# PhiFEM/phiFEM

Measured on AMD Instinct MI355X. Metric: assembled+solved DoF/s, 3D Poisson phi-FEM (tag+assemble+solve), higher is better.
Workload: dtype f64

## Files before the change

include/phifem_hip.h:

```cpp
#ifndef PHIFEM_HIP_H
#define PHIFEM_HIP_H

#include <stdint.h>

#ifdef __cplusplus
extern "C" {
#endif

typedef struct phx_mesh phx_mesh;
typedef struct phx_system phx_system;

enum phx_status {
  PHX_OK = 0,
  PHX_ERR_VALUE = -1,
  PHX_ERR_NOT_IMPLEMENTED = -2,
  PHX_ERR_HIP = -3,
  PHX_ERR_PARTITION = -4,
  PHX_ERR_CAPACITY = -5,
  PHX_ERR_BREAKDOWN = -6,
  PHX_ERR_TIMEOUT = -7
};

enum phx_loc { PHX_HOST = 0, PHX_DEVICE = 1 };

// ... 15 lines not shown
  PHX_ARR_BFACETS = 6,
  PHX_ARR_C2E = 7,
  PHX_ARR_EDGES = 8
};

int phx_version(void);
const char *phx_last_error(void);
int phx_device_count(int *n);
int phx_pool_release(void);
int phx_pool_stats(int64_t *live_bytes, int64_t *cached_bytes);

int phx_detection_points(int cell_type, int degree, int which, double *out, int64_t *npts);

int phx_levelset_points_count(phx_mesh *m, int detection_degree, int64_t *count);
int phx_levelset_eval_points(phx_mesh *m, int detection_degree, const double *nodal, int loc,
                             double *out_device);
int phx_detection_points_physical(phx_mesh *m, int detection_degree, double *out_device);

int phx_lagrange_nodes(int cell_type, int degree, double *out, int64_t *n);
int phx_lagrange_tabulate(int cell_type, int degree, int64_t npts, const double *pts, double *out);
int phx_levelset_eval_points_deg(phx_mesh *m, int detection_degree, int levelset_degree, const double *nodal,
                                 int loc, double *out_device);
int phx_lagrange_dof_points(phx_mesh *m, int degree, double *out_device);

int phx_topology_build_host(int cell_type, int64_t nv, int64_t nc, const int32_t *cells,
                            int32_t *c2f, int32_t *f2c, int64_t *nf);

int phx_mesh_create(int gdim, int cell_type, int64_t nv, const double *coords, int64_t nc,
                    const int32_t *cells, int device, phx_mesh **out);

int phx_mesh_create_box(int gdim, const double *lo, const double *hi, const int64_t *n,
                        const int64_t *offset, const int64_t *n_global, int device,
                        phx_mesh **out);

int phx_mesh_set_slab_faces(phx_mesh *m, int lower_is_cut, int upper_is_cut);
int phx_mesh_destroy(phx_mesh *m);
int phx_mesh_edge_count(phx_mesh *m, int64_t *ne);
int phx_mesh_counts(const phx_mesh *m, int64_t *counts);
int phx_mesh_get_array(phx_mesh *m, int which, void *out, int loc);
int phx_mesh_stream(phx_mesh *m, uint64_t *stream);
int phx_mesh_synchronize(phx_mesh *m);
int phx_mesh_set_stream(phx_mesh *m, uint64_t stream);
enum phx_option {
  PHX_OPT_PROFILE_SPMV = 1,
  PHX_OPT_HAS_EXTERIOR = 2,
  PHX_OPT_SPMV_XCD_GROUP = 3,
  PHX_OPT_PRECOND = 5,
  PHX_OPT_EXPORT_CSR = 7,
  PHX_OPT_STRUCTURED = 8,
  PHX_OPT_DETERMINISTIC = 9,
  PHX_OPT_EL_COARSE = 10,
  PHX_OPT_STENCIL_PLANE_ROWS = 11,
  PHX_OPT_P2_COARSE = 12,
  PHX_OPT_ALLOW_EMPTY = 6,
  PHX_OPT_SPMV_VALUE_INDEX = 4
};
int phx_set_option(phx_mesh *m, int option, int64_t value);
int phx_box_poisson_solve(int device, const int *L, const double *h, int f32, double *f_host);
int phx_box_dst_bench(int device, const int *L, int f32, int reps, double *out_us3);
int phx_dense_inverse(int device, int64_t n, double *a_host, int *singular);
int phx_event_pair_overhead(phx_mesh *m, double *seconds);
int phx_mesh_tag_histogram(const phx_mesh *m, int64_t *cells4, int64_t *facets7);

int phx_tag_cells(phx_mesh *m, int phi_kind, const double *phi, int loc, int detection_degree,
                  int single_layer_cut, int *warn_zero_denominator);

int phx_tag_facets(phx_mesh *m, int phi_kind, const double *phi, int loc, int detection_degree);

int phx_overwrite_tags(phx_mesh *m, int entity_is_facet, int64_t n, const int32_t *indices,
                       const int32_t *values);
int phx_set_tags(phx_mesh *m, int entity_is_facet, const int32_t *values, int loc);

int phx_integration_entities(phx_mesh *m, int which, int32_t *out, int64_t *n_pairs);

int phx_submesh_create(phx_mesh *m, phx_mesh **sub);
int phx_submesh_maps(phx_mesh *sub, int32_t *c_map, int32_t *v_map);

int phx_partition_cells(phx_mesh *m, int nparts, const int32_t *weights, int32_t *part, int loc);
int phx_partition_layout(phx_mesh *m, int nparts, const int32_t *part, int rank, int32_t *owner, uint8_t *flags, int loc);
int phx_submesh_create_from_flags(phx_mesh *m, const uint8_t *flags, int loc, phx_mesh **sub);

int phx_mesh_refine(phx_mesh *m, phx_mesh **fine);
int phx_prolongate(phx_mesh *coarse, phx_mesh *fine, int degree, int ncomp, const double *in, int loc_in,
                   double *out, int loc_out);
int phx_refine_tables(int cell_type, int32_t *children, int *nchild, double *p2_weights);

int phx_locate_points(phx_mesh *m, int64_t npts, const double *pts, int loc, double tol, int32_t *cells_out,
                      double *xref_out, int loc_out);
int phx_eval_points(phx_mesh *m, int degree, int ncomp, const double *values, int loc_v, int64_t npts,
                    const int32_t *cells, const double *xref, int loc_p, int want_grad, double fill, double *out,
                    double *grad_out, int loc_out);
int phx_locator_info(const phx_mesh *m, int64_t *info);
int phx_locate_timings(const phx_mesh *m, double *t);

int phx_assemble_poisson_wd(phx_mesh *m, double pen_coef, double stab_coef, const double *phi_h,
                            const double *f_h, const double *u_D, int loc, phx_system **out);
int phx_assemble_poisson_wd_p2(phx_mesh *m, double pen_coef, double stab_coef, const double *phi_h,
                               int phi_degree, const double *f_h, const double *u_D, int loc,
                               phx_system **out);
int phx_assemble_poisson_sd(phx_mesh *m, double stab_coef, int degree, const double *phi_h,
                            int phi_degree, const double *f_h, int loc, phx_system **out);
int phx_assemble_poisson_flux(phx_mesh *m, const double *params, int facet_tag, int quadrature_degree,
                              const double *phi_h, const double *f_h, const double *g_h, int loc,
                              phx_system **out);
int phx_assemble_elasticity_if(phx_mesh *m, const double *params, const double *phi_h,
                               const double *f_h, const double *u_D, const int32_t *bc_vertices,
// ... 61 lines not shown
```

phifem_amd/_lib.py:

```python
import ctypes as C
import os

_HERE = os.path.dirname(os.path.abspath(__file__))
LIB_PATH = os.path.join(_HERE, "libphifem_hip.so")

if not os.path.exists(LIB_PATH):
    raise ImportError(
        f"{LIB_PATH} is missing: build it with `python -c 'import __graft_entry__ as g; g.build()'` "
        "(or `make -C phifem_amd/csrc`).  phifem_amd has no CPU fallback.")

if os.environ.get("PHIFEM_NO_TORCH", "") != "1":
    try:
        import torch
    except ImportError:
        pass

lib = C.CDLL(LIB_PATH)

HOST, DEVICE = 0, 1
TRIANGLE, QUADRILATERAL, TETRAHEDRON = 0, 1, 2
CELL_TYPES = {"triangle": TRIANGLE, "quadrilateral": QUADRILATERAL, "tetrahedron": TETRAHEDRON}
CELL_NAMES = {v: k for k, v in CELL_TYPES.items()}
PHI_NODAL_P1, PHI_POINTS, PHI_QUADRIC = 0, 1, 2
(OPT_PROFILE_SPMV, OPT_HAS_EXTERIOR, OPT_SPMV_XCD_GROUP, OPT_SPMV_VALUE_INDEX, OPT_PRECOND, OPT_ALLOW_EMPTY,
 OPT_EXPORT_CSR, OPT_STRUCTURED, OPT_DETERMINISTIC, OPT_EL_COARSE, OPT_STENCIL_PLANE_ROWS, OPT_P2_COARSE) = (
    1, 2, 3, 4, 5, 6, 7, 8, 9, 10, 11, 12)
(ARR_COORDS, ARR_CELLS, ARR_C2F, ARR_F2C, ARR_CELL_TAGS, ARR_FACET_TAGS, ARR_BFACETS, ARR_C2E,
 ARR_EDGES) = range(9)

OK, ERR_VALUE, ERR_NOT_IMPLEMENTED, ERR_HIP, ERR_PARTITION, ERR_CAPACITY, ERR_BREAKDOWN, ERR_TIMEOUT = (
    0, -1, -2, -3, -4, -5, -6, -7)

_vp, _i, _i64, _d = C.c_void_p, C.c_int, C.c_int64, C.c_double
_pi, _pi64, _pd = C.POINTER(C.c_int), C.POINTER(C.c_int64), C.POINTER(C.c_double)

SIGNATURES = {
    "phx_version": ([], _i),
    "phx_last_error": ([], C.c_char_p),
    "phx_device_count": ([_pi], _i),
    "phx_pool_release": ([], _i),
    "phx_pool_stats": ([_pi64, _pi64], _i),
    "phx_detection_points": ([_i, _i, _i, _vp, _pi64], _i),
    "phx_levelset_points_count": ([_vp, _i, _pi64], _i),
    "phx_levelset_eval_points": ([_vp, _i, _vp, _i, _vp], _i),
    "phx_detection_points_physical": ([_vp, _i, _vp], _i),
    "phx_lagrange_nodes": ([_i, _i, _vp, _pi64], _i),
    "phx_lagrange_tabulate": ([_i, _i, _i64, _vp, _vp], _i),
    "phx_levelset_eval_points_deg": ([_vp, _i, _i, _vp, _i, _vp], _i),
    "phx_lagrange_dof_points": ([_vp, _i, _vp], _i),
    "phx_topology_build_host": ([_i, _i64, _i64, _vp, _vp, _vp, _pi64], _i),
    "phx_mesh_create": ([_i, _i, _i64, _vp, _i64, _vp, _i, C.POINTER(_vp)], _i),
    "phx_mesh_create_box": ([_i, _vp, _vp, _vp, _vp, _vp, _i, C.POINTER(_vp)], _i),
    "phx_mesh_set_slab_faces": ([_vp, _i, _i], _i),
    "phx_mesh_destroy": ([_vp], _i),
    "phx_mesh_counts": ([_vp, _pi64], _i),
    "phx_mesh_edge_count": ([_vp, _pi64], _i),
    "phx_mesh_get_array": ([_vp, _i, _vp, _i], _i),
    "phx_mesh_stream": ([_vp, C.POINTER(C.c_uint64)], _i),
    "phx_mesh_synchronize": ([_vp], _i),
    "phx_mesh_set_stream": ([_vp, C.c_uint64], _i),
    "phx_set_option": ([_vp, _i, _i64], _i),
    "phx_event_pair_overhead": ([_vp, _pd], _i),
    "phx_box_poisson_solve": ([_i, _pi, _pd, _i, _vp], _i),
    "phx_box_dst_bench": ([_i, _pi, _i, _i, _pd], _i),
    "phx_mesh_tag_histogram": ([_vp, _pi64, _pi64], _i),
    "phx_krylov_precond_active": ([_vp, _pi], _i),
    "phx_krylov_precond_disable": ([_vp], _i),
    "phx_precond_info": ([_vp, _pd], _i),
    "phx_coarse_info": ([_vp, _pd], _i),
    "phx_coarse_export": ([_vp, _vp, _vp], _i),
    "phx_precond_local_bbox": ([_vp, _pi64], _i),
    "phx_precond_setup_global": ([_vp, _pi64, _i, _i, _pi64, _pi64], _i),
    "phx_precond_set_carry_buffers": ([_vp, _vp, _vp], _i),
    "phx_precond_dist_info": ([_vp, _pi64], _i),
    "phx_krylov_attach": ([_vp, _vp, _vp, _vp], _i),
    "phx_krylov_phase": ([_vp, _i], _i),
    "phx_krylov_finish": ([_vp, _vp, _i], _i),
    "phx_krylov_profile": ([_vp, _i, _pd, _pi64], _i),
    "phx_system_get_perm": ([_vp, _vp, _vp, _vp, _i], _i),
# ... 96 lines not shown
```

phifem_amd/csrc/phx_common.h:

```cpp
#pragma once
#include <hip/hip_runtime.h>
#include <stdint.h>
#include <stdio.h>
#include <string>
#include <vector>

#include "../../include/phifem_hip.h"
#include "phx_switches.h"

#define PHX_MAX_PTS 40
#define PHX_MAX_VPC 4

void phx_set_error(const char *fmt, ...);

hipError_t phx_pool_malloc(void **p, size_t bytes);
hipError_t phx_pool_free(void *p);
void phx_pool_trim(void);
template <typename T>
static inline hipError_t phx_malloc(T **p, size_t bytes) { return phx_pool_malloc((void **)p, bytes); }
static inline hipError_t phx_free(void *p) { return phx_pool_free(p); }

#define PHX_HIP(expr)                                                                       \
  do {                                                                                      \
    hipError_t e_ = (expr);                                                                 \
// ... 57 lines not shown
  int32_t *bfacets = nullptr;
  int32_t *bfacet_ids = nullptr;
  uint8_t *facet_exempt = nullptr;
  bool slab_cut = false;
  int64_t ne = 0;
  int32_t *c2e = nullptr;
  int32_t *edges = nullptr;
  bool c2e_is_alias = false;
  int64_t box_n[3] = {0, 0, 0};
  double box_h[3] = {0.0, 0.0, 0.0};
  int64_t box_off[3] = {0, 0, 0};
  int64_t box_nglob[3] = {0, 0, 0};
  double box_lo[3] = {0.0, 0.0, 0.0}, box_hi[3] = {0.0, 0.0, 0.0};
  int64_t *v2c_ptr = nullptr;
  int32_t *v2c_idx = nullptr;
  bool is_box = false;
  int64_t box_plane = 0, box_nlast = 0;
  int8_t *cell_tags = nullptr;
  int8_t *facet_tags = nullptr;
  bool have_cell_tags = false, have_facet_tags = false;
  int64_t tag_hist[4] = {0, 0, 0, 0};
  int64_t ftag_hist[8] = {0, 0, 0, 0, 0, 0, 0, 0};
  int32_t *sel_counts[2] = {nullptr, nullptr};
  bool sel_counts_valid = false;
  int64_t sel_total[2] = {0, 0};
  int32_t *sel_counts_cut = nullptr;
  bool sel_cut_valid = false;
  uint8_t *act_in = nullptr, *act_cut = nullptr;
  bool act_valid = false;
  int64_t *ent_buf[2] = {nullptr, nullptr};
  int64_t ent_count[2] = {0, 0};
  bool have_entities = false;
  bool is_submesh = false;
  int32_t *c_map_h = nullptr, *v_map_h = nullptr;
  bool on_box_lattice = false;
  int32_t *v2lat = nullptr;
  int32_t *lat2v = nullptr;
  double timings[8] = {0, 0, 0, 0, 0, 0, 0, 0};
  struct phx_locator *locator = nullptr;
  int rect_checked = 0;
  double loc_timings[3] = {0, 0, 0};
  bool own_stream = true;
  int profile_spmv = 0;
  int spmv_xcd_group = 0;
  int64_t stencil_plane_rows = 32768;
  int spmv_value_index = 1;
  int precond = 1;
  int has_exterior_override = -1;
  std::vector<hipEvent_t> prof_ev[2];
  int prof_used[2] = {0, 0}, prof_seen[2] = {0, 0};
  double *scal_h = nullptr;
  int export_csr = 0;
  int structured = 1;
  int allow_empty = 0;
  int el_coarse = -1;
  int p2_coarse = 0;
  int deterministic = 0;
  phx_mesh *inner = nullptr;
  int32_t *in_cmap = nullptr;
  int32_t *in_fmap = nullptr;
};

struct phx_p2_lattice {
  int64_t n[3];
  int64_t F[3];
  int64_t nv;
  int64_t base[8];
  int64_t ext[7][3];
};
__host__ __device__ __forceinline__ int phx_p2_edge_class(int a, int b, int c) {
  const int nd = a + b + c;
  return nd == 1 ? (a ? 0 : (b ? 1 : 2)) : (nd == 2 ? (!c ? 3 : (!b ? 4 : 5)) : 6);
}
__host__ __device__ __forceinline__ int64_t phx_p2_entity_of_fine(const phx_p2_lattice &L, int64_t I, int64_t J, int64_t K) {
  const int a = (int)(I & 1), b = (int)(J & 1), c = (int)(K & 1);
  const int64_t i = I >> 1, j = J >> 1, k = K >> 1;
  if (!(a | b | c)) return i + (L.n[0] + 1) * (j + (L.n[1] + 1) * k);
  const int cls = phx_p2_edge_class(a, b, c);
  return L.nv + L.base[cls] + i + L.ext[cls][0] * (j + L.ext[cls][1] * k);
}
__host__ __device__ __forceinline__ void phx_p2_fine_of_entity(const phx_p2_lattice &L, int64_t e, int64_t *q) {
  if (e < L.nv) {
    const int64_t n0 = L.n[0] + 1, n1 = L.n[1] + 1, r = e / n0;
    q[0] = 2 * (e - r * n0); q[1] = 2 * (r % n1); q[2] = 2 * (r / n1);
    return;
  }
  const int64_t id = e - L.nv;
  int cls = 0;
  while (cls < 6 && id >= L.base[cls + 1]) ++cls;
  const int64_t rem = id - L.base[cls], r = rem / L.ext[cls][0];
  const int dir[7][3] = {{1, 0, 0}, {0, 1, 0}, {0, 0, 1}, {1, 1, 0}, {1, 0, 1}, {0, 1, 1}, {1, 1, 1}};
  q[0] = 2 * (rem - r * L.ext[cls][0]) + dir[cls][0];
  q[1] = 2 * (r % L.ext[cls][1]) + dir[cls][1];
  q[2] = 2 * (r / L.ext[cls][1]) + dir[cls][2];
}
#define PHX_P2S_REC 32
struct phx_p2_struct {
  phx_p2_lattice lat;
  double *coef = nullptr;
  unsigned long long *mask = nullptr;
  double *tabE = nullptr, *tabO = nullptr;
  unsigned *linemask = nullptr;
  int32_t *runs = nullptr;
  int64_t nrun = 0, nc0i = 0;
};

// ... 109 lines not shown
```

phifem_amd/csrc/phx_mesh.hip:

```cpp
#include "phx_prim.h"
#include <stdarg.h>
#include <string.h>

#include <algorithm>
#include <atomic>
#include <vector>

#include "phx_common.h"
#include "phx_select.h"

static thread_local char g_err[1024] = "";

void phx_set_error(const char *fmt, ...) {
  va_list ap;
  va_start(ap, fmt);
  vsnprintf(g_err, sizeof(g_err), fmt, ap);
  va_end(ap);
}

#include <map>
#include <mutex>
#include <unordered_map>
namespace {
struct Pool {
// ... 1059 lines not shown
  }
  RbArgs a;
  memset(&a, 0, sizeof(a));
  a.n = n;
  int tot = 0;
  for (int i = 0; i < n; ++i) {
    PHX_REQUIRE(items[i].bytes > 0 && items[i].bytes <= 64, PHX_ERR_VALUE, "read-back item of %d bytes", items[i].bytes);
    a.src[i] = static_cast<const uint8_t *>(items[i].dev);
    a.bytes[i] = items[i].bytes;
    a.off[i] = tot;
    tot += (items[i].bytes + 7) & ~7;
  }
  k_rb_pack<<<1, 64, 0, st>>>(a, sg.dev);
  PHX_HIP(hipGetLastError());
  PHX_HIP(hipMemcpyAsync(sg.pin, sg.dev, (size_t)tot, hipMemcpyDeviceToHost, st));
  PHX_HIP(hipStreamSynchronize(st));
  for (int i = 0; i < n; ++i) memcpy(items[i].host, sg.pin + a.off[i], (size_t)items[i].bytes);
  return PHX_OK;
}

int phx_mesh_pinned_scalars(phx_mesh *m, double **out) {
  if (!m->scal_h) PHX_HIP(hipHostMalloc(&m->scal_h, sizeof(double) * 16));
  *out = m->scal_h;
  return PHX_OK;
}

extern "C" int phx_mesh_stream(phx_mesh *m, uint64_t *stream) {
  *stream = (uint64_t)(uintptr_t)m->stream;
  return PHX_OK;
}

extern "C" int phx_mesh_set_stream(phx_mesh *m, uint64_t stream) {
  PHX_HIP(hipSetDevice(m->device));
  PHX_HIP(hipStreamSynchronize(m->stream));
  if (m->own_stream) PHX_HIP(hipStreamDestroy(m->stream));
  m->stream = (hipStream_t)(uintptr_t)stream;
  m->own_stream = false;
  if (m->inner) m->inner->stream = m->stream;
  return PHX_OK;
}

extern "C" int phx_set_option(phx_mesh *m, int option, int64_t value) {
  if (m->inner) PHX_CHECK(phx_set_option(m->inner, option, value));
  switch (option) {
    case PHX_OPT_PROFILE_SPMV:
      PHX_REQUIRE(value >= 0 && value <= 1024, PHX_ERR_VALUE, "SpMV profiling stride out of range");
      m->profile_spmv = (int)value;
      return PHX_OK;
    case PHX_OPT_HAS_EXTERIOR: m->has_exterior_override = (int)value; return PHX_OK;
    case PHX_OPT_SPMV_VALUE_INDEX: m->spmv_value_index = value != 0; return PHX_OK;
    case PHX_OPT_ALLOW_EMPTY: m->allow_empty = value != 0; return PHX_OK;
    case PHX_OPT_EXPORT_CSR: m->export_csr = value != 0; return PHX_OK;
    case PHX_OPT_STRUCTURED: m->structured = value != 0; return PHX_OK;
    case PHX_OPT_DETERMINISTIC: m->deterministic = value != 0; return PHX_OK;
    case PHX_OPT_EL_COARSE:
      PHX_REQUIRE(value == -1 || value == 0 || (value >= 5 && value <= 4096), PHX_ERR_VALUE, "coarse ratio %lld: -1, 0 or >= 5", (long long)value);
      m->el_coarse = (int)value;
      return PHX_OK;
    case PHX_OPT_P2_COARSE:
      PHX_REQUIRE(value == -1 || value == 0 || (value >= 5 && value <= 4096), PHX_ERR_VALUE, "coarse ratio %lld: -1, 0 or >= 5", (long long)value);
      m->p2_coarse = (int)value;
      return PHX_OK;
    case PHX_OPT_PRECOND:
      PHX_REQUIRE(value >= 0 && value <= 2, PHX_ERR_VALUE, "unknown preconditioner %lld", (long long)value);
      m->precond = (int)value;
      return PHX_OK;
    case PHX_OPT_SPMV_XCD_GROUP:
      PHX_REQUIRE(value >= 0 && value < (1 << 24), PHX_ERR_VALUE, "XCD group size out of range");
      m->spmv_xcd_group = (int)value;
      return PHX_OK;
    case PHX_OPT_STENCIL_PLANE_ROWS:
      PHX_REQUIRE(value >= 0, PHX_ERR_VALUE, "rows per plane out of range");
      m->stencil_plane_rows = value;
      return PHX_OK;
    default: phx_set_error("unknown option %d", option); return PHX_ERR_VALUE;
  }
}

extern "C" int phx_mesh_tag_histogram(const phx_mesh *m, int64_t *cells4, int64_t *facets7) {
  if (cells4) for (int i = 0; i < 4; ++i) cells4[i] = m->tag_hist[i];
  if (facets7) for (int i = 0; i < 7; ++i) facets7[i] = m->ftag_hist[i];
  return PHX_OK;
}

extern "C" int phx_mesh_synchronize(phx_mesh *m) {
  PHX_HIP(hipSetDevice(m->device));
  PHX_HIP(hipStreamSynchronize(m->stream));
  return PHX_OK;
}

__global__ void k_widen_tags(int64_t n, const int8_t *__restrict__ in, int32_t *__restrict__ out) {
  const int64_t i = blockIdx.x * (int64_t)blockDim.x + threadIdx.x;
  if (i < n) out[i] = (int32_t)(in[i] & PHX_TAG_MASK);
}

extern "C" int phx_mesh_get_array(phx_mesh *m, int which, void *out, int loc) {
  PHX_HIP(hipSetDevice(m->device));
  const hipMemcpyKind kind = loc == PHX_DEVICE ? hipMemcpyDeviceToDevice : hipMemcpyDeviceToHost;
  const void *src = nullptr;
  size_t bytes = 0;
  switch (which) {
    case PHX_ARR_COORDS: src = m->x; bytes = sizeof(double) * m->nv * m->gdim; break;
    case PHX_ARR_CELLS: src = m->cells; bytes = sizeof(int32_t) * m->nc * m->ci.nvpc; break;
    case PHX_ARR_C2F: src = m->c2f; bytes = sizeof(int32_t) * m->nc * m->ci.nfpc; break;
    case PHX_ARR_F2C: src = m->f2c; bytes = sizeof(int32_t) * m->nf * 2; break;
    case PHX_ARR_BFACETS: src = m->bfacets; bytes = sizeof(int32_t) * m->nbf * 2; break;
// ... 36 lines not shown
```

phifem_amd/csrc/phx_tag.hip:

```cpp
#include "phx_prim.h"
#include <string.h>

#include <algorithm>
#include <vector>

#include "phx_common.h"
#include "phx_select.h"

int phx_shape_table(int cell_type, int degree, int which, std::vector<double> &tab, int *npts,
                    int *nfun);

struct DetTab {
  int npts, nfun;
  double N[PHX_MAX_PTS * 4];
};
struct Quadric {
  double c[3], s[3], c0;
};
struct FacetVerts {
  int nfpc, nvpf;
  int fv[4][3];
};

template <int GDIM>
// ... 323 lines not shown
  unsigned long long a = 0;
  for (int64_t i = blockIdx.x * (int64_t)blockDim.x + threadIdx.x; i < nblocks; i += (int64_t)gridDim.x * blockDim.x)
    a += part[(size_t)b * nblocks + i];
  red[threadIdx.x] = a;
  __syncthreads();
  for (int o = 128; o > 0; o >>= 1) {
    if ((int)threadIdx.x < o) red[threadIdx.x] += red[threadIdx.x + o];
    __syncthreads();
  }
  if (threadIdx.x == 0 && red[0]) atomicAdd(&hist[b], red[0]);
}

struct SelTag34 {
  const int8_t *ft;
  __host__ __device__ bool operator()(const int32_t &f) const { return ft[f] == 3 || ft[f] == 4; }
  __host__ __device__ const int8_t *bytes() const { return ft; }
  __host__ __device__ bool test(int t, int32_t) const { return t == 3 || t == 4; }
};

template <bool FILL>
__global__ void k_entities(int64_t nlist, const int32_t *__restrict__ list,
                           const int32_t *__restrict__ f2c, const int32_t *__restrict__ c2f,
                           int nfpc, const int8_t *__restrict__ ctags,
                           const int8_t *__restrict__ ftags, int32_t *__restrict__ cnt0,
                           int32_t *__restrict__ cnt1, const int32_t *__restrict__ off0,
                           const int32_t *__restrict__ off1, int64_t *__restrict__ out0,
                           int64_t *__restrict__ out1) {
  const int64_t i = blockIdx.x * (int64_t)blockDim.x + threadIdx.x;
  if (i >= nlist) return;
  const int64_t f = list[i];
  const int w = ftags[f] == 4 ? 0 : 1;
  const int cell_mask = w == 0 ? ((1 << 1) | (1 << 2)) : ((1 << 2) | (1 << 3));
  const int32_t c0 = f2c[2 * f], c1 = f2c[2 * f + 1];
  int n = 0;
  for (int pos = 0; pos < 2; ++pos) {
    const int32_t c = c1 >= 0 ? (pos == 0 ? c1 : c0) : (pos == 0 ? c0 : -1);
    if (c < 0) continue;
    const int t = ctags[c] & PHX_TAG_MASK;
    if (t > 30 || !((cell_mask >> t) & 1)) continue;
    if (FILL) {
      int lf = 0;
      for (int k = 0; k < nfpc; ++k)
        if (c2f[(int64_t)c * nfpc + k] == (int32_t)f) lf = k;
      int64_t *out = w == 0 ? out0 : out1;
      const int64_t slot = (w == 0 ? off0[i] : off1[i]) + n;
      out[2 * slot] = 2 * f + pos;
      out[2 * slot + 1] = ((int64_t)c << 8) | lf;
    }
    ++n;
  }
  if (!FILL) { cnt0[i] = w == 0 ? n : 0; cnt1[i] = w == 1 ? n : 0; }
}

static int make_tab(const phx_mesh *m, int degree, int which, DetTab *tab) {
  std::vector<double> t;
  int npts = 0, nfun = 0;
  PHX_CHECK(phx_shape_table(m->cell_type, degree, which, t, &npts, &nfun));
  memset(tab, 0, sizeof(*tab));
  tab->npts = npts;
  tab->nfun = nfun;
  for (size_t i = 0; i < t.size(); ++i) tab->N[i] = t[i];
  return PHX_OK;
}

static int stage_phi(phx_mesh *m, int phi_kind, const double *phi, int loc, int64_t count,
                     const double **dev, double **owned, Quadric *quad) {
  *owned = nullptr;
  *dev = nullptr;
  memset(quad, 0, sizeof(*quad));
  PHX_REQUIRE(phi != nullptr, PHX_ERR_VALUE, "phi is NULL");
  if (phi_kind == PHX_PHI_QUADRIC) {
    double h[7];
    if (loc == PHX_DEVICE) PHX_HIP(hipMemcpy(h, phi, sizeof(h), hipMemcpyDeviceToHost));
    else memcpy(h, phi, sizeof(h));
    for (int a = 0; a < 3; ++a) { quad->c[a] = h[a]; quad->s[a] = h[3 + a]; }
    quad->c0 = h[6];
    return PHX_OK;
  }
  if (loc == PHX_DEVICE) { *dev = phi; return PHX_OK; }
  PHX_HIP(phx_malloc(owned, sizeof(double) * (size_t)(count > 0 ? count : 1)));
  PHX_HIP(hipMemcpyAsync(*owned, phi, sizeof(double) * (size_t)count, hipMemcpyHostToDevice, m->stream));
  *dev = *owned;
  return PHX_OK;
}

static int64_t cell_points_count(const phx_mesh *m, int degree) {
  DetTab t;
  if (make_tab(m, degree, 0, &t) != PHX_OK) return 0;
  return t.npts;
}

static int read_hist(phx_mesh *m, const int8_t *tags, int64_t n, int nbins, int64_t *out, const void *extra = nullptr,
                     size_t extra_bytes = 0, void *extra_host = nullptr) {
  unsigned long long *d = nullptr;
  PHX_HIP(phx_malloc(&d, sizeof(unsigned long long) * 8));
  PHX_HIP(hipMemsetAsync(d, 0, sizeof(unsigned long long) * 8, m->stream));
  const int blocks = (int)std::min<int64_t>(phx_div_up(n, 256), 2048);
  k_tag_hist<<<dim3(blocks), dim3(256), 0, m->stream>>>(n, tags, nbins, d);
  unsigned long long h[8];
  const phx_rb_item rb[2] = {{d, (int)sizeof(h), h}, {extra, (int)extra_bytes, extra_host}};
  PHX_CHECK(phx_read_back(m->stream, rb, extra ? 2 : 1));
  PHX_HIP(phx_free(d));
  for (int i = 0; i < nbins; ++i) out[i] = (int64_t)h[i];
  return PHX_OK;
}

template <int KIND>
static int launch_tag_cells(phx_mesh *m, const DetTab &tab, const double *dphi, const Quadric &q,
                            int *dwarn) {
  const dim3 grid((unsigned)phx_div_up(m->nc, 256)), block(256);
  if (m->cell_type == PHX_TRIANGLE)
    k_tag_cells<KIND, 2, 3><<<grid, block, 0, m->stream>>>(m->nc, tab, m->cells, dphi, m->x, q, m->cell_tags, dwarn);
  else if (m->cell_type == PHX_QUADRILATERAL)
    k_tag_cells<KIND, 2, 4><<<grid, block, 0, m->stream>>>(m->nc, tab, m->cells, dphi, m->x, q, m->cell_tags, dwarn);
  else
    k_tag_cells<KIND, 3, 4><<<grid, block, 0, m->stream>>>(m->nc, tab, m->cells, dphi, m->x, q, m->cell_tags, dwarn);
  PHX_HIP(hipGetLastError());
  return PHX_OK;
}

extern "C" int phx_tag_cells(phx_mesh *m, int phi_kind, const double *phi, int loc,
                             int detection_degree, int single_layer_cut,
                             int *warn_zero_denominator) {
  PHX_HIP(hipSetDevice(m->device));
  PHX_REQUIRE(phi_kind >= 0 && phi_kind <= 2, PHX_ERR_VALUE, "unknown phi_kind %d", phi_kind);
  DetTab tab;
  PHX_CHECK(make_tab(m, detection_degree, 0, &tab));
  const double *dphi = nullptr;
  double *owned = nullptr;
  Quadric quad;
  const int64_t count = phi_kind == PHX_PHI_NODAL_P1 ? m->nv : m->nc * (int64_t)tab.npts;
  PHX_CHECK(stage_phi(m, phi_kind, phi, loc, count, &dphi, &owned, &quad));
  int *dwarn = nullptr;
  PHX_HIP(phx_malloc(&dwarn, sizeof(int)));
  PHX_HIP(hipMemsetAsync(dwarn, 0, sizeof(int), m->stream));
  PHX_CHECK(phx_begin_timing(m));
  if (phi_kind == PHX_PHI_NODAL_P1) PHX_CHECK(launch_tag_cells<PHX_PHI_NODAL_P1>(m, tab, dphi, quad, dwarn));
  else if (phi_kind == PHX_PHI_POINTS) PHX_CHECK(launch_tag_cells<PHX_PHI_POINTS>(m, tab, dphi, quad, dwarn));
  else PHX_CHECK(launch_tag_cells<PHX_PHI_QUADRIC>(m, tab, dphi, quad, dwarn));
  uint8_t *touched = nullptr, *vcut = nullptr;
  const dim3 grid4((unsigned)phx_div_up(phx_div_up(m->nc, 4), 256)), block4(256);
  m->act_valid = false;
  if (single_layer_cut) {
    if (!m->act_in) PHX_HIP(phx_malloc(&m->act_in, (size_t)m->nv));
    if (!m->act_cut) PHX_HIP(phx_malloc(&m->act_cut, (size_t)m->nv));
    touched = m->act_in;
    vcut = m->act_cut;
    PHX_HIP(hipMemsetAsync(vcut, 0, (size_t)m->nv, m->stream));
    PHX_HIP(hipMemsetAsync(touched, 0, (size_t)m->nv, m->stream));
    if (m->ci.nvpc == 3) k_mark_inside_vertices<3><<<grid4, block4, 0, m->stream>>>(m->nc, m->cells, m->cell_tags, touched);
    else k_mark_inside_vertices<4><<<grid4, block4, 0, m->stream>>>(m->nc, m->cells, m->cell_tags, touched);
  }
  unsigned long long *dres = nullptr;
  uint32_t *part = nullptr;
  const int64_t nchunks = phx_div_up(m->nc > 0 ? m->nc : 1, (int64_t)PHX_SEL_CHUNK);
  PHX_HIP(phx_malloc(&dres, sizeof(unsigned long long) * 4));
  PHX_HIP(phx_malloc(&part, sizeof(uint32_t) * 4 * (size_t)grid4.x));
  PHX_HIP(hipMemsetAsync(dres, 0, sizeof(unsigned long long) * 4, m->stream));
  if (!m->sel_counts_cut) PHX_HIP(phx_malloc(&m->sel_counts_cut, sizeof(int32_t) * (size_t)(nchunks + 1)));
  PHX_HIP(hipMemsetAsync(m->sel_counts_cut, 0, sizeof(int32_t) * (size_t)(nchunks + 1), m->stream));
  if (m->ci.nvpc == 3) k_demote_isolated_cut<3><<<grid4, block4, 0, m->stream>>>(m->nc, m->cells, m->cell_tags, touched, part, m->sel_counts_cut, vcut);
  else k_demote_isolated_cut<4><<<grid4, block4, 0, m->stream>>>(m->nc, m->cells, m->cell_tags, touched, part, m->sel_counts_cut, vcut);
  PHX_HIP(hipGetLastError());
  PHX_CHECK(phx_end_timing_mark(m));
  k_hist_fold<<<dim3(64, 4), dim3(256), 0, m->stream>>>((int64_t)grid4.x, part, dres);
  int hwarn = 0;
  unsigned long long hh[4] = {0, 0, 0, 0};
  const phx_rb_item rb[2] = {{dres, (int)sizeof(hh), hh}, {dwarn, (int)sizeof(int), &hwarn}};
  PHX_CHECK(phx_read_back(m->stream, rb, 2));
  for (int i = 0; i < 4; ++i) m->tag_hist[i] = (int64_t)hh[i];
  m->sel_cut_valid = true;
  m->act_valid = single_layer_cut != 0;
  PHX_CHECK(phx_end_timing_read(m, 0));
  PHX_HIP(phx_free(dres));
  PHX_HIP(phx_free(part));
  PHX_HIP(phx_free(dwarn));
  if (owned) PHX_HIP(phx_free(owned));
  if (warn_zero_denominator) *warn_zero_denominator = hwarn;
  m->have_cell_tags = true;
  m->have_facet_tags = false;
  m->sel_counts_valid = false;
  m->have_entities = false;
  return PHX_OK;
}

template <int KIND>
static int launch_bcut(phx_mesh *m, const DetTab &tab, const FacetVerts &fvs, const double *dphi,
                       const Quadric &q) {
  if (m->nbf == 0) return PHX_OK;
  const dim3 grid((unsigned)phx_div_up(m->nbf, 256)), block(256);
  if (m->gdim == 2)
    k_boundary_cell_cut<KIND, 2><<<grid, block, 0, m->stream>>>(m->nbf, tab, fvs, m->ci.nvpc, m->bfacets, m->bfacet_ids, m->cells, m->c2f, m->f2c, dphi, m->x, q, m->facet_exempt, m->cell_tags);
  else
    k_boundary_cell_cut<KIND, 3><<<grid, block, 0, m->stream>>>(m->nbf, tab, fvs, m->ci.nvpc, m->bfacets, m->bfacet_ids, m->cells, m->c2f, m->f2c, dphi, m->x, q, m->facet_exempt, m->cell_tags);
  PHX_HIP(hipGetLastError());
  return PHX_OK;
}

__global__ void k_clear_bcut(int64_t n, int8_t *tags) {
  const int64_t i0 = (blockIdx.x * (int64_t)blockDim.x + threadIdx.x) * 4;
  if (i0 + 3 < n) {
    uint32_t *w = reinterpret_cast<uint32_t *>(tags + i0);
    *w &= 0x01010101u * (uint32_t)PHX_TAG_MASK;
  } else {
    for (int64_t i = i0; i < n; ++i) tags[i] = (int8_t)(tags[i] & PHX_TAG_MASK);
  }
}

static int run_facet_rule(phx_mesh *m) {
  unsigned long long *dbad = nullptr;
  uint32_t *part = nullptr;
  const int64_t nblocks = phx_div_up(phx_div_up(m->nf, 4), 256);
  const int64_t nchunks = phx_div_up(m->nf > 0 ? m->nf : 1, (int64_t)PHX_SEL_CHUNK);
  PHX_HIP(phx_malloc(&dbad, sizeof(unsigned long long) * 10));
  PHX_HIP(phx_malloc(&part, sizeof(uint32_t) * 9 * (size_t)nblocks));
  PHX_HIP(hipMemsetAsync(dbad, 0, sizeof(unsigned long long) * 10, m->stream));
  for (int w = 0; w < 2; ++w) {
    if (!m->sel_counts[w]) PHX_HIP(phx_malloc(&m->sel_counts[w], sizeof(int32_t) * (size_t)(nchunks + 1)));
// ... 231 lines not shown
```

Measured before the change: 114.2 million.

## Add structured-box fast path for tetrahedral cell tagging

Adds box-specific kernels for the tag-cells path on structured 3D tetrahedral box meshes. Each thread handles one cube and its six tets, computing vertex indices arithmetically instead of reading the cell connectivity. Phi is loaded once per cube and shared across the six tets, and tag writes are coalesced through shared memory. The mark-inside and demote/count kernels are rewritten the same way, and the path is on by default behind a new option. This relies on the generated box mesh ordering six tets per cube with a fixed corner permutation, which is a correctness risk if that ordering ever differs.

Measured after the change: 116.3 million (median of 6 runs). 1.02x the previous value.

```diff
diff --git a/include/phifem_hip.h b/include/phifem_hip.h
--- a/include/phifem_hip.h
+++ b/include/phifem_hip.h
@@ -91,6 +91,7 @@
   PHX_OPT_EL_COARSE = 10,
   PHX_OPT_STENCIL_PLANE_ROWS = 11,
   PHX_OPT_P2_COARSE = 12,
+  PHX_OPT_BOX_TAGS = 13,
   PHX_OPT_ALLOW_EMPTY = 6,
   PHX_OPT_SPMV_VALUE_INDEX = 4
 };
diff --git a/phifem_amd/_lib.py b/phifem_amd/_lib.py
--- a/phifem_amd/_lib.py
+++ b/phifem_amd/_lib.py
@@ -23,8 +23,9 @@
 CELL_NAMES = {v: k for k, v in CELL_TYPES.items()}
 PHI_NODAL_P1, PHI_POINTS, PHI_QUADRIC = 0, 1, 2
 (OPT_PROFILE_SPMV, OPT_HAS_EXTERIOR, OPT_SPMV_XCD_GROUP, OPT_SPMV_VALUE_INDEX, OPT_PRECOND, OPT_ALLOW_EMPTY,
- OPT_EXPORT_CSR, OPT_STRUCTURED, OPT_DETERMINISTIC, OPT_EL_COARSE, OPT_STENCIL_PLANE_ROWS, OPT_P2_COARSE) = (
-    1, 2, 3, 4, 5, 6, 7, 8, 9, 10, 11, 12)
+ OPT_EXPORT_CSR, OPT_STRUCTURED, OPT_DETERMINISTIC, OPT_EL_COARSE, OPT_STENCIL_PLANE_ROWS, OPT_P2_COARSE,
+ OPT_BOX_TAGS) = (
+    1, 2, 3, 4, 5, 6, 7, 8, 9, 10, 11, 12, 13)
 (ARR_COORDS, ARR_CELLS, ARR_C2F, ARR_F2C, ARR_CELL_TAGS, ARR_FACET_TAGS, ARR_BFACETS, ARR_C2E,
  ARR_EDGES) = range(9)
 
diff --git a/phifem_amd/csrc/phx_common.h b/phifem_amd/csrc/phx_common.h
--- a/phifem_amd/csrc/phx_common.h
+++ b/phifem_amd/csrc/phx_common.h
@@ -133,6 +133,7 @@
   double *scal_h = nullptr;
   int export_csr = 0;
   int structured = 1;
+  int box_tags = 1;
   int allow_empty = 0;
   int el_coarse = -1;
   int p2_coarse = 0;
diff --git a/phifem_amd/csrc/phx_mesh.hip b/phifem_amd/csrc/phx_mesh.hip
--- a/phifem_amd/csrc/phx_mesh.hip
+++ b/phifem_amd/csrc/phx_mesh.hip
@@ -1135,6 +1135,7 @@
     case PHX_OPT_ALLOW_EMPTY: m->allow_empty = value != 0; return PHX_OK;
     case PHX_OPT_EXPORT_CSR: m->export_csr = value != 0; return PHX_OK;
     case PHX_OPT_STRUCTURED: m->structured = value != 0; return PHX_OK;
+    case PHX_OPT_BOX_TAGS: m->box_tags = value != 0; return PHX_OK;
     case PHX_OPT_DETERMINISTIC: m->deterministic = value != 0; return PHX_OK;
     case PHX_OPT_EL_COARSE:
       PHX_REQUIRE(value == -1 || value == 0 || (value >= 5 && value <= 4096), PHX_ERR_VALUE, "coarse ratio %lld: -1, 0 or >= 5", (long long)value);
diff --git a/phifem_amd/csrc/phx_tag.hip b/phifem_amd/csrc/phx_tag.hip
--- a/phifem_amd/csrc/phx_tag.hip
+++ b/phifem_amd/csrc/phx_tag.hip
@@ -399,6 +399,8 @@
   if (!FILL) { cnt0[i] = w == 0 ? n : 0; cnt1[i] = w == 1 ? n : 0; }
 }
 
+#include "phx_tag_box.inc.hip"
+
 static int make_tab(const phx_mesh *m, int degree, int which, DetTab *tab) {
   std::vector<double> t;
   int npts = 0, nfun = 0;
@@ -482,7 +484,14 @@
   PHX_HIP(phx_malloc(&dwarn, sizeof(int)));
   PHX_HIP(hipMemsetAsync(dwarn, 0, sizeof(int), m->stream));
   PHX_CHECK(phx_begin_timing(m));
-  if (phi_kind == PHX_PHI_NODAL_P1) PHX_CHECK(launch_tag_cells<PHX_PHI_NODAL_P1>(m, tab, dphi, quad, dwarn));
+  const bool box = box_tags_apply(m);
+  BoxTagGeo bg;
+  dim3 bgrid, bblock;
+  if (box) box_tag_launch_dims(m, &bg, &bgrid, &bblock);
+  if (box && phi_kind == PHX_PHI_NODAL_P1) {
+    k_box_tag_cells<<<bgrid, bblock, 0, m->stream>>>(bg, tab, dphi, m->x, m->cell_tags, dwarn);
+    PHX_HIP(hipGetLastError());
+  } else if (phi_kind == PHX_PHI_NODAL_P1) PHX_CHECK(launch_tag_cells<PHX_PHI_NODAL_P1>(m, tab, dphi, quad, dwarn));
   else if (phi_kind == PHX_PHI_POINTS) PHX_CHECK(launch_tag_cells<PHX_PHI_POINTS>(m, tab, dphi, quad, dwarn));
   else PHX_CHECK(launch_tag_cells<PHX_PHI_QUADRIC>(m, tab, dphi, quad, dwarn));
   uint8_t *touched = nullptr, *vcut = nullptr;
@@ -495,22 +504,25 @@
     vcut = m->act_cut;
     PHX_HIP(hipMemsetAsync(vcut, 0, (size_t)m->nv, m->stream));
     PHX_HIP(hipMemsetAsync(touched, 0, (size_t)m->nv, m->stream));
-    if (m->ci.nvpc == 3) k_mark_inside_vertices<3><<<grid4, block4, 0, m->stream>>>(m->nc, m->cells, m->cell_tags, touched);
+    if (box) k_box_mark_inside<<<bgrid, bblock, 0, m->stream>>>(bg, m->cell_tags, touched);
+    else if (m->ci.nvpc == 3) k_mark_inside_vertices<3><<<grid4, block4, 0, m->stream>>>(m->nc, m->cells, m->cell_tags, touched);
     else k_mark_inside_vertices<4><<<grid4, block4, 0, m->stream>>>(m->nc, m->cells, m->cell_tags, touched);
   }
   unsigned long long *dres = nullptr;
   uint32_t *part = nullptr;
   const int64_t nchunks = phx_div_up(m->nc > 0 ? m->nc : 1, (int64_t)PHX_SEL_CHUNK);
   PHX_HIP(phx_malloc(&dres, sizeof(unsigned long long) * 4));
-  PHX_HIP(phx_malloc(&part, sizeof(uint32_t) * 4 * (size_t)grid4.x));
+  const int64_t npart = box ? (int64_t)bgrid.x * bgrid.y * bgrid.z : (int64_t)grid4.x;
+  PHX_HIP(phx_malloc(&part, sizeof(uint32_t) * 4 * (size_t)npart));
   PHX_HIP(hipMemsetAsync(dres, 0, sizeof(unsigned long long) * 4, m->stream));
   if (!m->sel_counts_cut) PHX_HIP(phx_malloc(&m->sel_counts_cut, sizeof(int32_t) * (size_t)(nchunks + 1)));
   PHX_HIP(hipMemsetAsync(m->sel_counts_cut, 0, sizeof(int32_t) * (size_t)(nchunks + 1), m->stream));
-  if (m->ci.nvpc == 3) k_demote_isolated_cut<3><<<grid4, block4, 0, m->stream>>>(m->nc, m->cells, m->cell_tags, touched, part, m->sel_counts_cut, vcut);
+  if (box) k_box_demote_count<<<bgrid, bblock, 0, m->stream>>>(bg, m->cell_tags, touched, part, m->sel_counts_cut, vcut);
+  else if (m->ci.nvpc == 3) k_demote_isolated_cut<3><<<grid4, block4, 0, m->stream>>>(m->nc, m->cells, m->cell_tags, touched, part, m->sel_counts_cut, vcut);
   else k_demote_isolated_cut<4><<<grid4, block4, 0, m->stream>>>(m->nc, m->cells, m->cell_tags, touched, part, m->sel_counts_cut, vcut);
   PHX_HIP(hipGetLastError());
   PHX_CHECK(phx_end_timing_mark(m));
-  k_hist_fold<<<dim3(64, 4), dim3(256), 0, m->stream>>>((int64_t)grid4.x, part, dres);
+  k_hist_fold<<<dim3(64, 4), dim3(256), 0, m->stream>>>(npart, part, dres);
   int hwarn = 0;
   unsigned long long hh[4] = {0, 0, 0, 0};
   const phx_rb_item rb[2] = {{dres, (int)sizeof(hh), hh}, {dwarn, (int)sizeof(int), &hwarn}};
diff --git a/phifem_amd/csrc/phx_tag_box.inc.hip b/phifem_amd/csrc/phx_tag_box.inc.hip
--- /dev/null
+++ b/phifem_amd/csrc/phx_tag_box.inc.hip
@@ -0,0 +1,228 @@
+struct BoxTagGeo {
+  int n0, n1, n2;
+  int64_t s1, s2;
+};
+
+__device__ __forceinline__ constexpr int box_tet_corner(int t, int m) {
+  constexpr int P[6][3] = {{0, 1, 2}, {0, 2, 1}, {1, 0, 2}, {1, 2, 0}, {2, 0, 1}, {2, 1, 0}};
+  return m == 0 ? 0 : (m == 1 ? (1 << P[t][0]) : (m == 2 ? ((1 << P[t][0]) | (1 << P[t][1])) : 7));
+}
+__device__ __forceinline__ constexpr uint32_t box_tet_corners(int t) {
+  return (1u << box_tet_corner(t, 0)) | (1u << box_tet_corner(t, 1)) | (1u << box_tet_corner(t, 2)) |
+         (1u << box_tet_corner(t, 3));
+}
+__device__ __forceinline__ uint32_t box_corner_mask(uint32_t tm) {
+  uint32_t m = 0;
+#pragma unroll
+  for (int t = 0; t < 6; ++t)
+    if ((tm >> t) & 1u) m |= box_tet_corners(t);
+  return m;
+}
+__device__ __forceinline__ int64_t box_corner_vertex(const BoxTagGeo &g, int64_t o, int b) {
+  return o + (b & 1) + ((b >> 1) & 1) * g.s1 + (b >> 2) * g.s2;
+}
+
+__device__ __forceinline__ int box_tet_classify(const DetTab &tab, const double ph[4], const int64_t v[4],
+                                                const double *__restrict__ x, double num, double den, bool mixed,
+                                                bool *zero_den) {
+  const double den0 = den;
+  if (mixed) {
+    double e[3][3];
+    for (int a = 0; a < 3; ++a)
+      for (int dd = 0; dd < 3; ++dd) e[a][dd] = x[v[a + 1] * 3 + dd] - x[v[0] * 3 + dd];
+    const double c0 = e[1][1] * e[2][2] - e[1][2] * e[2][1];
+    const double c1 = e[1][0] * e[2][2] - e[1][2] * e[2][0];
+    const double c2 = e[1][0] * e[2][1] - e[1][1] * e[2][0];
+    const double s = fabs((e[0][0] * c0 - e[0][1] * c1) + e[0][2] * c2);
+    num = 0.0;
+    den = 0.0;
+    for (int q = 0; q < tab.npts; ++q) {
+      const double *N = &tab.N[q * tab.nfun];
+      double p = N[0] * ph[0];
+      for (int i = 1; i < 4; ++i) p = p + N[i] * ph[i];
+      const double t = p * s;
+      num = num + t;
+      den = den + fabs(t);
+    }
+  }
+  const double d = (den > 0.0) ? num / den : 0.5;
+  int t = 0;
+  if (d > -1.0 && d < 1.0) t = 2;
+  if (d == 1.0) t = 3;
+  if (d == -1.0) t = 1;
+  *zero_den = *zero_den || fabs(den0) <= 1.0e-8;
+  return t;
+}
+
+__global__ void __launch_bounds__(256)
+k_box_tag_cells(BoxTagGeo g, DetTab tab, const double *__restrict__ phi, const double *__restrict__ x,
+                int8_t *__restrict__ tags, int *__restrict__ warn) {
+  __shared__ uint32_t st[4][98];
+  const int lane = threadIdx.x & 63, wv = threadIdx.x >> 6;
+  const int i = (int)(blockIdx.x * blockDim.x + threadIdx.x);
+  const int j = (int)blockIdx.y, k = (int)blockIdx.z;
+  const int64_t row = (int64_t)g.n0 * (j + (int64_t)g.n1 * k);
+  const int wi0 = i - lane;
+  const int64_t B = 6 * (row + wi0);
+  const int pad = (int)(B & 3);
+  uint16_t *st16 = reinterpret_cast<uint16_t *>(st[wv]);
+  if (i < g.n0) {
+    const int64_t o = i + g.s1 * j + g.s2 * k;
+    double pv[8];
+#pragma unroll
+    for (int b = 0; b < 8; ++b) pv[b] = phi[box_corner_vertex(g, o, b)];
+    double num[6], den[6];
+    uint32_t pos = 0, neg = 0;
+#pragma unroll
+    for (int t = 0; t < 6; ++t) num[t] = den[t] = 0.0;
+    for (int q = 0; q < tab.npts; ++q) {
+      const double *N = &tab.N[q * tab.nfun];
+      const double N0 = N[0], N1 = N[1], N2 = N[2], N3 = N[3];
+#pragma unroll
+      for (int t = 0; t < 6; ++t) {
+        double p = N0 * pv[box_tet_corner(t, 0)];
+        p = p + N1 * pv[box_tet_corner(t, 1)];
+        p = p + N2 * pv[box_tet_corner(t, 2)];
+        p = p + N3 * pv[box_tet_corner(t, 3)];
+        num[t] = num[t] + p;
+        den[t] = den[t] + fabs(p);
+        pos |= (uint32_t)(p > 0.0) << t;
+        neg |= (uint32_t)(p < 0.0) << t;
+      }
+    }
+    bool zero_den = false;
+    uint32_t tg[6];
+#pragma unroll
+    for (int t = 0; t < 6; ++t) {
+      const double ph[4] = {pv[box_tet_corner(t, 0)], pv[box_tet_corner(t, 1)], pv[box_tet_corner(t, 2)],
+                            pv[box_tet_corner(t, 3)]};
+      const int64_t v[4] = {box_corner_vertex(g, o, box_tet_corner(t, 0)), box_corner_vertex(g, o, box_tet_corner(t, 1)),
+                            box_corner_vertex(g, o, box_tet_corner(t, 2)), box_corner_vertex(g, o, box_tet_corner(t, 3))};
+      tg[t] = (uint32_t)box_tet_classify(tab, ph, v, x, num[t], den[t], ((pos & neg) >> t) & 1u, &zero_den);
+    }
+    if (zero_den) atomicOr(warn, 1);
+    const int h = (pad >> 1) + 3 * lane;
+    st16[h] = (uint16_t)(tg[0] | (tg[1] << 8));
+    st16[h + 1] = (uint16_t)(tg[2] | (tg[3] << 8));
+    st16[h + 2] = (uint16_t)(tg[4] | (tg[5] << 8));
+  }
+  __syncthreads();
+  if (wi0 >= g.n0) return;
+  const int nvalid = min(64, g.n0 - wi0);
+  const int64_t A = B + pad;
+  const int nbytes = 6 * nvalid - pad;
+  const int nd = nbytes >> 2, first = pad >> 1;
+  uint32_t *g32 = reinterpret_cast<uint32_t *>(tags);
+  uint16_t *g16 = reinterpret_cast<uint16_t *>(tags);
+  for (int w = lane; w < nd; w += 64) g32[(A >> 2) + w] = st[wv][first + w];
+  if (lane == 0 && pad) g16[B >> 1] = st16[1];
+  if (lane == 1 && (nbytes & 2)) g16[(A >> 1) + 2 * nd] = st16[2 * (first + nd)];
+}
+
+__device__ __forceinline__ void box_load_tags(const int8_t *tags, int64_t cube, int t[6]) {
+  const uint16_t *t16 = reinterpret_cast<const uint16_t *>(tags) + 3 * cube;
+#pragma unroll
+  for (int h = 0; h < 3; ++h) {
+    const uint32_t w = t16[h];
+    t[2 * h] = (int)(w & PHX_TAG_MASK);
+    t[2 * h + 1] = (int)((w >> 8) & PHX_TAG_MASK);
+  }
+}
+
+__global__ void __launch_bounds__(256)
+k_box_mark_inside(BoxTagGeo g, const int8_t *__restrict__ tags, uint8_t *__restrict__ touched) {
+  const int i = (int)(blockIdx.x * blockDim.x + threadIdx.x);
+  if (i >= g.n0) return;
+  const int j = (int)blockIdx.y, k = (int)blockIdx.z;
+  const int64_t cube = i + (int64_t)g.n0 * (j + (int64_t)g.n1 * k);
+  int t[6];
+  box_load_tags(tags, cube, t);
+  uint32_t tm = 0;
+#pragma unroll
+  for (int s = 0; s < 6; ++s) tm |= (uint32_t)(t[s] == 1) << s;
+  if (!tm) return;
+  const uint32_t cm = box_corner_mask(tm);
+  const int64_t o = i + g.s1 * j + g.s2 * k;
+#pragma unroll
+  for (int b = 0; b < 8; ++b)
+    if ((cm >> b) & 1u) touched[box_corner_vertex(g, o, b)] = 1;
+}
+
+__global__ void __launch_bounds__(256)
+k_box_demote_count(BoxTagGeo g, int8_t *__restrict__ tags, const uint8_t *__restrict__ touched,
+                   uint32_t *__restrict__ hist_part, int32_t *__restrict__ sel_cut, uint8_t *__restrict__ vcut) {
+  __shared__ uint32_t lh[4][4];
+  const int lane = threadIdx.x & 63, wv = threadIdx.x >> 6;
+  const int i = (int)(blockIdx.x * blockDim.x + threadIdx.x);
+  const int j = (int)blockIdx.y, k = (int)blockIdx.z;
+  const int64_t row = (int64_t)g.n0 * (j + (int64_t)g.n1 * k);
+  const int64_t cube = row + i;
+  int t[6] = {0x7f, 0x7f, 0x7f, 0x7f, 0x7f, 0x7f};
+  if (i < g.n0) {
+    box_load_tags(tags, cube, t);
+    uint32_t tm = 0;
+#pragma unroll
+    for (int s = 0; s < 6; ++s) tm |= (uint32_t)(t[s] == 2) << s;
+    if (tm && touched) {
+      const uint32_t cm = box_corner_mask(tm);
+      const int64_t o = i + g.s1 * j + g.s2 * k;
+      uint32_t in = 0;
+#pragma unroll
+      for (int b = 0; b < 8; ++b)
+        if ((cm >> b) & 1u) in |= (uint32_t)(touched[box_corner_vertex(g, o, b)] != 0) << b;
+      uint32_t stay = 0;
+#pragma unroll
+      for (int s = 0; s < 6; ++s) {
+        if (!((tm >> s) & 1u)) continue;
+        if (in & box_tet_corners(s)) stay |= box_tet_corners(s);
+        else { tags[6 * cube + s] = 3; t[s] = 3; }
+      }
+      if (vcut) {
+#pragma unroll
+        for (int b = 0; b < 8; ++b)
+          if ((stay >> b) & 1u) vcut[box_corner_vertex(g, o, b)] = 1;
+      }
+    }
+  }
+  const int wi0 = i - lane;
+  const int64_t wbase = 6 * (row + wi0);
+  const int64_t bnd = (wbase / PHX_SEL_CHUNK + 1) * (int64_t)PHX_SEL_CHUNK;
+  uint32_t cnt[4] = {0, 0, 0, 0}, lo = 0;
+#pragma unroll
+  for (int s = 0; s < 6; ++s) {
+#pragma unroll
+    for (int b = 0; b < 4; ++b) cnt[b] += (uint32_t)__popcll(__ballot(t[s] == b));
+    lo += (uint32_t)__popcll(__ballot(t[s] == 2 && 6 * cube + s < bnd));
+  }
+  if (lane == 0) {
+    if (wi0 < g.n0) {
+      const int64_t chunk = wbase / PHX_SEL_CHUNK;
+      if (lo) atomicAdd(&sel_cut[chunk], (int32_t)lo);
+      if (cnt[2] - lo) atomicAdd(&sel_cut[chunk + 1], (int32_t)(cnt[2] - lo));
+    }
+    for (int b = 0; b < 4; ++b) lh[wv][b] = cnt[b];
+  }
+  __syncthreads();
+  const int nw = (int)(blockDim.x >> 6);
+  if (threadIdx.x < 4) {
+    uint32_t a = 0;
+    for (int w = 0; w < nw; ++w) a += lh[w][threadIdx.x];
+    const size_t nblocks = (size_t)gridDim.x * gridDim.y * gridDim.z;
+    const size_t blk = blockIdx.x + (size_t)gridDim.x * (blockIdx.y + (size_t)gridDim.y * blockIdx.z);
+    hist_part[(size_t)threadIdx.x * nblocks + blk] = a;
+  }
+}
+
+static bool box_tags_apply(const phx_mesh *m) {
+  return m->box_tags != 0 && m->is_box && !m->is_submesh && m->gdim == 3 && m->cell_type == PHX_TETRAHEDRON &&
+         m->box_n[1] <= 65535 && m->box_n[2] <= 65535;
+}
+
+static void box_tag_launch_dims(const phx_mesh *m, BoxTagGeo *g, dim3 *grid, dim3 *block) {
+  g->n0 = (int)m->box_n[0]; g->n1 = (int)m->box_n[1]; g->n2 = (int)m->box_n[2];
+  g->s1 = m->box_n[0] + 1;
+  g->s2 = (m->box_n[0] + 1) * (m->box_n[1] + 1);
+  const int threads = (int)std::min<int64_t>(256, phx_div_up(m->box_n[0], 64) * 64);
+  *block = dim3((unsigned)threads);
+  *grid = dim3((unsigned)phx_div_up(m->box_n[0], threads), (unsigned)m->box_n[1], (unsigned)m->box_n[2]);
+}
```
